# meituan/YOLOv6

Measured on NVIDIA H100. Metric: images/sec YOLOv6-S 640 bs32, higher is better.
Workload: dtype bf16

## Files before the change

### include/yv6.h

```cpp
#ifndef YV6_H_
#define YV6_H_

#include <stdint.h>

#ifdef __cplusplus
extern "C" {
#endif

#define YV6_ABI_VERSION 4

enum {
  YV6_OK = 0,
  YV6_ERR_ARG = -1,
  YV6_ERR_CUDA = -2,
  YV6_ERR_STATE = -3
};

enum { YV6_ACT_NONE = 0, YV6_ACT_RELU = 1, YV6_ACT_SILU = 2, YV6_ACT_SIGMOID = 3 };
enum { YV6_DT_BF16 = 0, YV6_DT_F32 = 1, YV6_DT_U8 = 2 };
#define YV6_PAD_SAME (-1000000)

typedef struct yv6_handle yv6_handle;

int yv6_create(int device, yv6_handle** out);
int yv6_destroy(yv6_handle* h);
const char* yv6_last_error(void);
int yv6_abi_version(void);

typedef struct yv6_conv_desc {
  const void* x;
  int32_t N, H, W, Cin;
  int32_t x_c_total;
  int64_t x_plane_stride;
  const void* w;
  int64_t w_plane_stride;
  const float* bias;
  int32_t Cout, kh, kw, stride, pad;
  int32_t act;
  void* y;
  int32_t y_dtype;
  int64_t y_img_stride, y_h_stride, y_w_stride;
  int64_t y_plane_stride;
  const void* res;
  float alpha;
  int64_t res_img_stride, res_h_stride, res_w_stride, res_plane_stride;
  int32_t nsplit;
  int32_t force_bw, force_bh, force_bi, force_bn, force_stages, force_grid;
  int32_t force_direct;
  int32_t force_halo;
  int32_t pad_w, out_h, out_w;
  int32_t force_groups;
  void* trace;
  int32_t stride_w;
  int32_t force_pair;
  int32_t pair_view;
  int32_t reserved0;
} yv6_conv_desc;

int yv6_conv_fwd(yv6_handle* h, const yv6_conv_desc* d, void* stream);
int yv6_conv_plan(yv6_handle* h, const yv6_conv_desc* d, int32_t* out10);
int yv6_conv_plan_host(int num_sms, int max_smem_optin, int max_clusters, const yv6_conv_desc* d, int32_t* out12);

typedef struct yv6_stem_desc {
  const void* x;
  int32_t x_dtype;
  float in_scale;
  int32_t N, H, W;
  const float* w;
  const float* bias;
  int32_t Cout, act;
  void* y;
  int64_t y_plane_stride;
  int32_t nsplit;
  int32_t fp32_math;
  int32_t force_sync_loads;
} yv6_stem_desc;
int yv6_stem_fwd(yv6_handle* h, const yv6_stem_desc* d, void* stream);

int yv6_sppf_pool(yv6_handle* h, void* buf, int32_t N, int32_t H, int32_t W, int32_t C, int32_t c_total,
                  int32_t nsplit, int64_t plane_stride, void* stream);

int yv6_head_decode(yv6_handle* h, const float* cls, const float* reg, float* out, int32_t B, int32_t nc,
                    int32_t reg_ch, int32_t nl, const int32_t* lvl_h, const int32_t* lvl_w,
                    const float* lvl_stride, void* stream);

int64_t yv6_nms_workspace_bytes(int32_t B, int32_t A, int32_t nc, int32_t multi_label);
int yv6_nms_batched(yv6_handle* h, const float* pred, int32_t B, int32_t A, int32_t nc, float conf_thres,
                    double iou_thres, int32_t agnostic, int32_t multi_label, const uint8_t* class_mask,
                    int32_t max_det, float* out, int32_t* out_count, int32_t* out_src, int32_t* overflow,
                    void* workspace, int64_t workspace_bytes, void* stream);

int yv6_nms_batched_head(yv6_handle* h, const float* cls, const float* reg, int32_t B, int32_t nc, int32_t reg_ch, int32_t nl,
                         const int32_t* lvl_h, const int32_t* lvl_w, const float* lvl_stride, float conf_thres, double iou_thres,
                         int32_t agnostic, int32_t multi_label, const uint8_t* class_mask, int32_t max_det, float* out,
                         int32_t* out_count, int32_t* out_src, int32_t* overflow, void* workspace, int64_t workspace_bytes,
                         void* stream);

int yv6_eval_boxes(yv6_handle* h, const float* det, const int32_t* count, const float* meta, int32_t B, int32_t max_det,
                   float* out, void* stream);

typedef struct yv6_pr_state {
  int32_t max_images, max_det, nc, confusion;
  float* conf; float* cls;
  uint16_t* correct;
  int32_t* ndet;
  int32_t* nt; int32_t* npred;
  int32_t* matrix;
  int32_t* flags;
} yv6_pr_state;
#define YV6_PR_OUT_SIZE(nc) ((int64_t)(nc) * 3010 + (int64_t)(nc) + ((int64_t)(nc) + 1) * ((int64_t)(nc) + 1) + 8)
int64_t yv6_pr_workspace_bytes(int32_t max_images, int32_t max_det);
int yv6_pr_match(yv6_handle* h, const yv6_pr_state* st, const float* det, const int32_t* count, int32_t B, int32_t max_det,
                 const float* targets, int32_t n_targets, const float* meta, int32_t H, int32_t W, const float* iouv,
                 int32_t first_image, void* stream);
int yv6_pr_metric(yv6_handle* h, const yv6_pr_state* st, int32_t n_images, const double* px, const double* x101, void* workspace,
                  int64_t workspace_bytes, double* out, void* stream);

#define YV6_LB_GEO 8
int yv6_letterbox(yv6_handle* h, const uint8_t* src, const int32_t* geo, int32_t B, int32_t H, int32_t W, uint8_t* dst,
                  void* stream);
int yv6_rescale_boxes(yv6_handle* h, const float* det, const int32_t* count, const int32_t* geo, int32_t B, int32_t max_det,
                      int32_t H, int32_t W, float* out, void* stream);

#define YV6_AUG_JOB 8
typedef struct {
  int64_t org;
  int32_t pitch;
  int32_t y0, y1, x0, x1;
  int32_t pad;
} yv6_aug_tile;
typedef struct {
  double minv[2][6];
  double mix_r;
  yv6_aug_tile tile[2][4];
  int32_t ch[2], cw[2];
  int32_t ntile[2];
  int32_t mixup, hsv, flipud, fliplr;
  uint8_t lut[3][256];
} yv6_aug_sample;
// ... 145 lines not shown
```

### yolov6_b200/_lib.py

```python
import ctypes as C
import os
import threading

_HERE = os.path.dirname(os.path.abspath(__file__))
LIB_PATH = os.path.join(_HERE, "libyolov6_b200.so")

ACT_NONE, ACT_RELU, ACT_SILU, ACT_SIGMOID = 0, 1, 2, 3
DT_BF16, DT_F32, DT_U8 = 0, 1, 2
PAD_SAME = -1000000
ACT_CODES = {None: ACT_NONE, "none": ACT_NONE, "relu": ACT_RELU, "silu": ACT_SILU, "sigmoid": ACT_SIGMOID}


class ConvDesc(C.Structure):
    _fields_ = [
        ("x", C.c_void_p), ("N", C.c_int32), ("H", C.c_int32), ("W", C.c_int32), ("Cin", C.c_int32),
        ("x_c_total", C.c_int32), ("x_plane_stride", C.c_int64),
        ("w", C.c_void_p), ("w_plane_stride", C.c_int64), ("bias", C.c_void_p),
        ("Cout", C.c_int32), ("kh", C.c_int32), ("kw", C.c_int32), ("stride", C.c_int32), ("pad", C.c_int32),
        ("act", C.c_int32),
        ("y", C.c_void_p), ("y_dtype", C.c_int32),
        ("y_img_stride", C.c_int64), ("y_h_stride", C.c_int64), ("y_w_stride", C.c_int64),
        ("y_plane_stride", C.c_int64),
        ("res", C.c_void_p), ("alpha", C.c_float),
        ("res_img_stride", C.c_int64), ("res_h_stride", C.c_int64), ("res_w_stride", C.c_int64),
        ("res_plane_stride", C.c_int64),
        ("nsplit", C.c_int32),
        ("force_bw", C.c_int32), ("force_bh", C.c_int32), ("force_bi", C.c_int32), ("force_bn", C.c_int32),
        ("force_stages", C.c_int32), ("force_grid", C.c_int32), ("force_direct", C.c_int32), ("force_halo", C.c_int32),
        ("pad_w", C.c_int32), ("out_h", C.c_int32), ("out_w", C.c_int32), ("force_groups", C.c_int32),
        ("trace", C.c_void_p), ("stride_w", C.c_int32), ("force_pair", C.c_int32), ("pair_view", C.c_int32), ("reserved0", C.c_int32),
    ]


class StemDesc(C.Structure):
    _fields_ = [
        ("x", C.c_void_p), ("x_dtype", C.c_int32), ("in_scale", C.c_float),
        ("N", C.c_int32), ("H", C.c_int32), ("W", C.c_int32),
        ("w", C.c_void_p), ("bias", C.c_void_p),
        ("Cout", C.c_int32), ("act", C.c_int32),
        ("y", C.c_void_p), ("y_plane_stride", C.c_int64), ("nsplit", C.c_int32), ("fp32_math", C.c_int32),
        ("force_sync_loads", C.c_int32),
    ]


class LossDesc(C.Structure):
    _fields_ = [
        ("pred_scores", C.c_void_p), ("pred_distri", C.c_void_p), ("anc_points", C.c_void_p), ("strides", C.c_void_p),
        ("gt", C.c_void_p), ("gt_idx", C.c_void_p), ("fg", C.c_void_p), ("norm", C.c_void_p),
        ("B", C.c_int32), ("A", C.c_int32), ("G", C.c_int32), ("nc", C.c_int32), ("reg_ch", C.c_int32),
        ("iou_type", C.c_int32),
        ("w_cls", C.c_double), ("w_iou", C.c_double), ("w_dfl", C.c_double), ("grad_scale", C.c_double),
        ("grad_scores", C.c_void_p), ("grad_distri", C.c_void_p), ("out", C.c_void_p),
        ("workspace", C.c_void_p), ("workspace_bytes", C.c_int64), ("norm_gt_zero", C.c_int32),
    ]


class WgradDesc(C.Structure):
    _fields_ = [
        ("x", C.c_void_p), ("N", C.c_int32), ("H", C.c_int32), ("W", C.c_int32), ("Cin", C.c_int32), ("x_c_total", C.c_int32),
        ("dy", C.c_void_p), ("Cout", C.c_int32), ("dy_c_total", C.c_int32),
        ("kh", C.c_int32), ("kw", C.c_int32), ("stride", C.c_int32), ("pad", C.c_int32),
        ("dw", C.c_void_p), ("force_ksplit", C.c_int32), ("force_taps", C.c_int32),
    ]


class BnDesc(C.Structure):
    _fields_ = [
        ("nb", C.c_int32), ("act", C.c_int32), ("C", C.c_int32), ("pixels", C.c_int64),
        ("x", C.c_void_p * 3), ("x_pitch", C.c_int64 * 3),
        ("mean", C.c_void_p * 3), ("invstd", C.c_void_p * 3), ("scale", C.c_void_p * 3), ("shift", C.c_void_p * 3),
        ("y", C.c_void_p), ("y_pitch", C.c_int64),
        ("dy", C.c_void_p), ("dy_pitch", C.c_int64),
        ("s1", C.c_void_p), ("s2", C.c_void_p * 3),
        ("dx", C.c_void_p * 3), ("dx_pitch", C.c_int64 * 3), ("accumulate", C.c_int32 * 3),
        ("res", C.c_void_p), ("res_pitch", C.c_int64), ("res_alpha", C.c_float),
        ("dres", C.c_void_p), ("dres_pitch", C.c_int64), ("dalpha", C.c_void_p),
        ("res_alpha_dev", C.c_void_p),
        ("work", C.c_void_p), ("counter", C.c_void_p), ("coef", C.c_void_p), ("zeroed", C.c_int32), ("dres_assign", C.c_int32),
    ]


class BnStatsDesc(C.Structure):
    _fields_ = [
        ("nb", C.c_int32), ("C", C.c_int32), ("pixels", C.c_int64),
        ("x", C.c_void_p * 3), ("x_pitch", C.c_int64 * 3),
        ("sums", C.c_void_p), ("counter", C.c_void_p), ("zeroed", C.c_int32),
        ("gamma", C.c_void_p * 3), ("beta", C.c_void_p * 3),
        ("running_mean", C.c_void_p * 3), ("running_var", C.c_void_p * 3),
        ("stats", C.c_void_p * 3),
        ("eps", C.c_float), ("momentum", C.c_float),
    ]


class XformSeg(C.Structure):
    _fields_ = [
        ("dst", C.c_void_p), ("src", C.c_void_p),
        ("n", C.c_int32 * 4), ("ds", C.c_int32 * 4), ("ss", C.c_int32 * 4),
        ("dst_dtype", C.c_int32), ("src_dtype", C.c_int32),
    ]


class PrState(C.Structure):
    _fields_ = [
        ("max_images", C.c_int32), ("max_det", C.c_int32), ("nc", C.c_int32), ("confusion", C.c_int32),
        ("conf", C.c_void_p), ("cls", C.c_void_p), ("correct", C.c_void_p), ("ndet", C.c_void_p),
        ("nt", C.c_void_p), ("npred", C.c_void_p), ("matrix", C.c_void_p), ("flags", C.c_void_p),
    ]


XF_F32, XF_F64, XF_BF16 = 0, 1, 2
XFORM_CHUNK = 4096


# ... 128 lines not shown
```

### yolov6_b200/csrc/yv6_conv_igemm.cu

```cuda
#include <algorithm>
#include <cstdarg>

#include "yv6_common.cuh"
#include "yv6_handle.h"
#include "yv6_wgmma.cuh"

namespace yv6 {

constexpr int kConvThreads = 384;
constexpr int kMaxStages = 12;
constexpr int kTileRows = 128;

struct ConvKParams {
  int32_t BW, BH, BI, rows;
  int32_t tiles_w, tiles_h, tiles_i, tiles_n, num_tiles;
  int32_t N, Ho, Wo, Cout, BN;
  int32_t taps, kw, stride, stride_w, pad, pad_w, Cin;
  int32_t cin_blocks, kb_elems, kb_bytes, ksteps;
  int32_t sbo_bytes, layout_type;
  int32_t npairs;
  int32_t stages, a_stage_bytes, b_stage_bytes;
  int32_t act, y_dtype, out_planes, res_planes;
  void* y;
  int64_t y_img_stride, y_h_stride, y_w_stride, y_plane_stride;
  const __nv_bfloat16* res;
  float alpha;
  int64_t res_img_stride, res_h_stride, res_w_stride, res_plane_stride;
  const float* bias;
  int32_t halo, a_stages, b_stages, b_resident;
  int32_t skip_cb;
  int32_t a_region_bytes, b_region_bytes;
  int32_t cpair, m_tiles, b_rows;
  int32_t fast_act;
};

constexpr int kHaloW = 10, kHaloH = 18;
template <bool S2>
struct HaloGeom {
  static constexpr int W = S2 ? 9 : kHaloW, H = S2 ? 33 : kHaloH, KW = S2 ? 2 : 3, TAPS = S2 ? 6 : 9, SH = S2 ? 2 : 1;
  static constexpr int kBytes = W * H * 128;
  static constexpr int kStageBytes = ((kBytes + 1023) / 1024) * 1024;
};
constexpr int kMaxAStages = 6, kMaxBStages = 40;

__host__ __device__ constexpr int stage_pitch(int bn) { return bn + 4; }
__host__ __device__ constexpr int staging_bytes(int bn) { return kTileRows * stage_pitch(bn) * 4; }

__device__ __forceinline__ void tma_load_3d(void* dst, const CUtensorMap* m, uint64_t* bar, int c0,
                                            int c1, int c2) {
  asm volatile(
      "cp.async.bulk.tensor.3d.shared::cluster.global.tile.mbarrier::complete_tx::bytes"
      " [%0], [%1, {%3, %4, %5}], [%2];" ::"r"(smem_u32(dst)),
      "l"(reinterpret_cast<uint64_t>(m)), "r"(smem_u32(bar)), "r"(c0), "r"(c1), "r"(c2)
      : "memory");
}
__device__ __forceinline__ void tma_load_3d_mc(void* dst, const CUtensorMap* m, uint64_t* bar, int c0, int c1, int c2,
                                               uint16_t mask) {
  asm volatile(
      "cp.async.bulk.tensor.3d.shared::cluster.global.mbarrier::complete_tx::bytes.multicast::cluster"
      " [%0], [%1, {%3, %4, %5}], [%2], %6;" ::"r"(smem_u32(dst)),
      "l"(reinterpret_cast<uint64_t>(m)), "r"(smem_u32(bar)), "r"(c0), "r"(c1), "r"(c2), "h"(mask)
      : "memory");
}
__device__ __forceinline__ void warpgroup_bar_sync(int wg) {
  asm volatile("bar.sync %0, 128;" ::"r"(1 + wg) : "memory");
}
__device__ __forceinline__ void producer_regs() { asm volatile("setmaxnreg.dec.sync.aligned.u32 40;"); }
__device__ __forceinline__ void consumer_regs() { asm volatile("setmaxnreg.inc.sync.aligned.u32 232;"); }

struct TileCoord {
  int w0, h0, i0, n0;
};
__device__ __forceinline__ TileCoord decode_tile(const ConvKParams& p, int tile) {
  TileCoord t;
  int nt = tile % p.tiles_n;
  int m = tile / p.tiles_n;
  int tw = m % p.tiles_w;
  m /= p.tiles_w;
  int th = m % p.tiles_h;
  int ti = m / p.tiles_h;
  t.w0 = tw * p.BW;
  t.h0 = th * p.BH;
  t.i0 = ti * p.BI;
  t.n0 = nt * p.BN;
  return t;
}

__device__ __forceinline__ TileCoord decode_unit(const ConvKParams& p, int unit, int rank) {
  TileCoord t;
  const int nt = unit % p.tiles_n;
  int m = (unit / p.tiles_n) * 2 + rank;
  t.n0 = nt * p.BN;
  if (m >= p.m_tiles) {
    t.w0 = 0;
    t.h0 = 0;
    t.i0 = p.N;
    return t;
  }
  const int tw = m % p.tiles_w;
  m /= p.tiles_w;
  const int th = m % p.tiles_h;
  const int ti = m / p.tiles_h;
  t.w0 = tw * p.BW;
  t.h0 = th * p.BH;
  t.i0 = ti * p.BI;
  return t;
}

__constant__ int kPairA[6] = {0, 1, 2, 0, 1, 0};
__constant__ int kPairB[6] = {2, 1, 0, 1, 0, 0};

__device__ __forceinline__ uint32_t pack_bf16x2(float a, float b) {
  __nv_bfloat162 v = __floats2bfloat162_rn(a, b);
  return *reinterpret_cast<uint32_t*>(&v);
}
// ... 70 lines not shown
    }
  } else {
#pragma unroll
    for (int j = 0; j < 16; ++j) v[j] = __uint_as_float(r[j]);
  }
  if (p.act == YV6_ACT_RELU) {
#pragma unroll
    for (int j = 0; j < 16; ++j) v[j] = fmaxf(v[j], 0.f);
  } else if (p.act == YV6_ACT_SILU) {
    if (p.fast_act) {
#pragma unroll
      for (int j = 0; j < 16; ++j) {
        const float h = 0.5f * v[j];
        v[j] = fmaf(h, tanh_fast(h), h);
      }
    } else {
#pragma unroll
      for (int j = 0; j < 16; ++j) v[j] = v[j] * rcp_ftz(1.f + ex2_ftz(-1.4426950408889634f * v[j]));
    }
  } else if (p.act == YV6_ACT_SIGMOID) {
#pragma unroll
    for (int j = 0; j < 16; ++j) v[j] = rcp_ftz(1.f + ex2_ftz(-1.4426950408889634f * v[j]));
  }
  if (p.res != nullptr && valid && ncol > 0) {
    for (int pl = 0; pl < p.res_planes; ++pl) {
      const __nv_bfloat16* rp = p.res + pl * p.res_plane_stride + roff + n;
      if (ncol == 16 && ((reinterpret_cast<uintptr_t>(rp) & 15) == 0)) {
        const uint4 q0 = __ldg(reinterpret_cast<const uint4*>(rp));
        const uint4 q1 = __ldg(reinterpret_cast<const uint4*>(rp) + 1);
        const uint32_t w[8] = {q0.x, q0.y, q0.z, q0.w, q1.x, q1.y, q1.z, q1.w};
#pragma unroll
        for (int j = 0; j < 8; ++j) {
          const __nv_bfloat162 b2 = *reinterpret_cast<const __nv_bfloat162*>(&w[j]);
          v[2 * j] += p.alpha * __low2float(b2);
          v[2 * j + 1] += p.alpha * __high2float(b2);
        }
      } else {
#pragma unroll
        for (int j = 0; j < 16; ++j)
          if (j < ncol) v[j] += p.alpha * __bfloat162float(rp[j]);
      }
    }
  }
}

template <int BN, int KSTEPS>
__device__ __forceinline__ void mma_kblock(float (&acc)[2][BN / 2], uint64_t ad, uint32_t a_hi, uint64_t bd, uint32_t scale_d) {
  wgmma_fence();
#pragma unroll
  for (int k = 0; k < KSTEPS; ++k) {
    const uint32_t sd = k == 0 ? scale_d : 1u;
    Wgmma<BN, 0, 0>::mma(acc[0], ad + (uint64_t)(2 * k), bd + (uint64_t)(2 * k), sd);
    Wgmma<BN, 0, 0>::mma(acc[1], ad + (uint64_t)(a_hi + 2 * k), bd + (uint64_t)(2 * k), sd);
  }
  wgmma_commit();
}

template <int BN, int MODE, bool CP>
__global__ void __launch_bounds__(kConvThreads, 1)
conv_igemm_kernel(const __grid_constant__ CUtensorMap tmA, const __grid_constant__ CUtensorMap tmB, const ConvKParams p) {
  extern __shared__ uint8_t smem_raw[];
  const uint32_t raw_addr = smem_u32(smem_raw);
  uint8_t* smem = smem_raw + ((1024u - (raw_addr & 1023u)) & 1023u);
  uint8_t* sA = smem;
  uint8_t* sB = smem + (size_t)p.a_region_bytes;
  float* sC = reinterpret_cast<float*>(sB + (size_t)p.b_region_bytes);
  uint64_t* bars = reinterpret_cast<uint64_t*>(reinterpret_cast<uint8_t*>(sC) + staging_bytes(BN));
  uint64_t* full = bars;
  uint64_t* empty = bars + kMaxStages;
  uint64_t* a_full = empty + kMaxStages;
  uint64_t* a_empty = a_full + kMaxAStages;
  uint64_t* b_full = a_empty + kMaxAStages;
  uint64_t* b_empty = b_full + kMaxBStages;
  uint64_t* mma_turn = b_empty + kMaxBStages;

  const int warp = threadIdx.x >> 5;
  const int lane = threadIdx.x & 31;
  constexpr bool HALO = (MODE != 0);
  constexpr bool BRES = (MODE == 2 || MODE == 4);
  using HG = HaloGeom<(MODE >= 3)>;
  const int rank = CP ? (int)cluster_ctarank() : 0;
  const int unit0 = CP ? (int)(blockIdx.x >> 1) : (int)blockIdx.x;
  const int ustep = CP ? (int)(gridDim.x >> 1) : (int)gridDim.x;
  auto coord = [&](int unit) { return CP ? decode_unit(p, unit, rank) : decode_tile(p, unit); };
  auto load_b = [&](uint8_t* dst, uint64_t* bar, int k, int n0, int plane) {
    if (CP) tma_load_3d_mc(dst + rank * p.b_rows * p.kb_bytes, &tmB, bar, k, n0 + rank * p.b_rows, plane, 3);
    else tma_load_3d(dst, &tmB, bar, k, n0, plane);
  };

  if (warp == 0) {
    if (lane == 0) {
      tma_prefetch_desc(&tmA);
      tma_prefetch_desc(&tmB);
    }
    constexpr int kRingSlots = 2 * kMaxStages + 2 * kMaxAStages + 2 * kMaxBStages;
    for (int i = lane; i < kRingSlots + 2; i += 32) {
      const bool is_b_empty = (i >= kMaxStages && i < 2 * kMaxStages) || (i >= 2 * kMaxStages + 2 * kMaxAStages + kMaxBStages && i < kRingSlots);
      mbar_init(&bars[i], i >= kRingSlots ? 128u : (is_b_empty && CP) ? 2u : 1u);
    }
    static_assert((kRingSlots + 2) * sizeof(uint64_t) <= 1024, "barriers overflow their 1 KB of shared memory");
    fence_mbar_init();
  }
  if (CP) cluster_sync_all();
  else __syncthreads();

  const int kblocks = p.npairs * p.taps * p.cin_blocks;

  if (warp < 4) {
    producer_regs();
    if (warp == 0) {
      if constexpr (HALO) {
        int sa = 0, sb = 0;
        uint32_t pha = 0, phb = 0;
        bool first = true;
        const uint32_t a_tx = (uint32_t)HG::kBytes, b_tx = (uint32_t)(BN * 128);
        for (int tile = unit0; tile < p.num_tiles; tile += ustep) {
          const TileCoord t = coord(tile);
          int slot = 0;
          for (int pi = 0; pi < p.npairs; ++pi) {
            const int pa = kPairA[6 - p.npairs + pi], pb = kPairB[6 - p.npairs + pi];
            for (int cb = 0; cb < p.cin_blocks; ++cb) {
              mbar_wait(&a_empty[sa], pha ^ 1);
              if (elect_one()) {
                mbar_expect_tx(&a_full[sa], a_tx);
                tma_load_5d(sA + (size_t)sa * HG::kStageBytes, &tmA, &a_full[sa], cb * 64, t.w0 - 1, t.h0 * HG::SH - 1, t.i0, pa);
              }
              __syncwarp();
              if (++sa == p.a_stages) { sa = 0; pha ^= 1; }
              for (int tap = 0; tap < HG::TAPS; ++tap) {
                if (HG::SH == 2 && (tap % HG::KW) == 0 && cb < p.skip_cb) continue;
                if constexpr (BRES) {
                  if (first && elect_one()) {
                    mbar_expect_tx(&b_full[slot], b_tx);
                    load_b(sB + (size_t)slot * p.b_stage_bytes, &b_full[slot], tap * p.Cin + cb * 64, t.n0, pb);
                  }
                  __syncwarp();
                } else {
                  mbar_wait(&b_empty[sb], phb ^ 1);
                  if (elect_one()) {
                    mbar_expect_tx(&b_full[sb], b_tx);
                    load_b(sB + (size_t)sb * p.b_stage_bytes, &b_full[sb], tap * p.Cin + cb * 64, t.n0, pb);
                  }
                  __syncwarp();
                  if (++sb == p.b_stages) { sb = 0; phb ^= 1; }
                }
                ++slot;
              }
            }
          }
          first = false;
        }
      } else {
        int stage = 0;
        uint32_t phase = 0;
        const uint32_t tx = (uint32_t)(p.rows * p.kb_bytes + BN * p.kb_bytes);
        for (int tile = unit0; tile < p.num_tiles; tile += ustep) {
          const TileCoord t = coord(tile);
          for (int pi = 0; pi < p.npairs; ++pi) {
            const int pa = kPairA[6 - p.npairs + pi], pb = kPairB[6 - p.npairs + pi];
            for (int tap = 0; tap < p.taps; ++tap) {
              const int r = tap / p.kw, s = tap - r * p.kw;
              const int cx = t.w0 * p.stride_w + s - p.pad_w;
              const int cy = t.h0 * p.stride + r - p.pad;
              for (int cb = 0; cb < p.cin_blocks; ++cb) {
                mbar_wait(&empty[stage], phase ^ 1);
                if (elect_one()) {
                  mbar_expect_tx(&full[stage], tx);
                  tma_load_5d(sA + (size_t)stage * p.a_stage_bytes, &tmA, &full[stage], cb * p.kb_elems, cx, cy, t.i0, pa);
                  load_b(sB + (size_t)stage * p.b_stage_bytes, &full[stage], tap * p.Cin + cb * p.kb_elems, t.n0, pb);
                }
                __syncwarp();
                if (++stage == p.stages) {
                  stage = 0;
                  phase ^= 1;
                }
              }
            }
          }
        }
      }
    }
  } else {
    consumer_regs();
    const int wg = (warp >> 2) - 1;
    const int ct = (int)threadIdx.x - 128 * (wg + 1);
    const bool arrive_lane = ct == 0;
    auto release_b = [&](uint64_t* bar) {
      mbar_arrive(bar);
      if (CP) mbar_arrive_cluster(bar, (uint32_t)(rank ^ 1));
    };
    auto skip_stages = [](int& s, uint32_t& ph, int n, int ring) {
      s += n;
      ph ^= (uint32_t)(s / ring) & 1u;
      s %= ring;
    };
    float acc[2][BN / 2];
    const uint32_t a_base = smem_u32(sA) >> 4, b_base = smem_u32(sB) >> 4;
    const int num_tiles = p.num_tiles, ksteps = p.ksteps, nstages = p.stages;
    const int pcs = p.npairs * p.cin_blocks;
    const int b_tile = p.npairs * (p.cin_blocks * HG::TAPS - (HG::SH == 2 ? (HG::TAPS / HG::KW) * p.skip_cb : 0));
    int stage = 0;
    uint32_t phase = 0;
    int sa = 0, sb = 0;
    uint32_t pha = 0, phb = 0, turn_ph = 0;
    bool first = true;
    float* sCw = sC + wg * 64 * stage_pitch(BN);
    for (int tile = unit0 + wg * ustep; tile < num_tiles; tile += 2 * ustep) {
      if (tile != unit0) {
        if constexpr (HALO) {
          skip_stages(sa, pha, pcs, p.a_stages);
          if (!BRES) skip_stages(sb, phb, b_tile, p.b_stages);
        } else {
          skip_stages(stage, phase, kblocks, nstages);
        }
        mbar_wait(&mma_turn[wg], turn_ph);
        turn_ph ^= 1;
      }
      if constexpr (HALO) {
        const uint32_t row_bytes = (uint32_t)(HG::W * 128 * HG::SH);
        const uint64_t desc_a = wgmma_desc(16u, row_bytes, 1u);
        const uint64_t desc_b = wgmma_desc(16u, 1024u, 1u);
        const uint32_t halo_step = (uint32_t)HG::kStageBytes >> 4, b_step = (uint32_t)p.b_stage_bytes >> 4;
        const uint32_t a_hi = 8u * (row_bytes >> 4);
        const int skip_cb = p.skip_cb, cin_blocks = p.cin_blocks, b_stages = p.b_stages;
        int slot = 0;
        uint32_t started = 0;
        int prev_sb = -1, prev_sa = -1;
        for (int pc = 0; pc < pcs; ++pc) {
          mbar_wait(&a_full[sa], pha);
          const uint32_t a0 = a_base + (uint32_t)sa * halo_step;
          const bool skip_s0 = (HG::SH == 2) && (pc % cin_blocks) < skip_cb;
#pragma unroll
          for (int tap = 0; tap < HG::TAPS; ++tap) {
            if (HG::SH == 2 && (tap % HG::KW) == 0 && skip_s0) continue;
            const int bs = BRES ? slot : sb;
            if (!BRES || first) mbar_wait(&b_full[bs], BRES ? 0u : phb);
            const uint64_t ad = desc_a | (uint64_t)(a0 + (uint32_t)((tap / HG::KW) * HG::W + (tap % HG::KW)) * 8u);
            const uint64_t bd = desc_b | (uint64_t)(b_base + (uint32_t)bs * b_step);
            mma_kblock<BN, 4>(acc, ad, a_hi, bd, started);
            started = 1u;
            if (!BRES || prev_sa >= 0) {
              wgmma_wait<1>();
              if (arrive_lane) {
                if (!BRES && prev_sb >= 0) release_b(&b_empty[prev_sb]);
                if (prev_sa >= 0) mbar_arrive(&a_empty[prev_sa]);
              }
              prev_sa = -1;
            }
            if (!BRES) {
              prev_sb = sb;
              if (++sb == b_stages) { sb = 0; phb ^= 1; }
            }
            ++slot;
          }
          prev_sa = sa;
          if (++sa == p.a_stages) { sa = 0; pha ^= 1; }
        }
        mbar_arrive(&mma_turn[wg ^ 1]);
        wgmma_wait<0>();
        if (arrive_lane) {
          if (!BRES && prev_sb >= 0) release_b(&b_empty[prev_sb]);
          if (prev_sa >= 0) mbar_arrive(&a_empty[prev_sa]);
        }
      } else {
        const uint64_t desc = wgmma_desc(16u, (uint32_t)p.sbo_bytes, (uint32_t)p.layout_type);
        const uint32_t a_step = (uint32_t)p.a_stage_bytes >> 4, b_step = (uint32_t)p.b_stage_bytes >> 4;
        const uint32_t a_hi = (uint32_t)(64 * p.kb_bytes) >> 4;
        int prev = -1;
        for (int kb = 0; kb < kblocks; ++kb) {
          mbar_wait(&full[stage], phase);
          const uint64_t ad = desc | (uint64_t)(a_base + (uint32_t)stage * a_step);
          const uint64_t bd = desc | (uint64_t)(b_base + (uint32_t)stage * b_step);
          const uint32_t scale_d = (uint32_t)(kb != 0);
          switch (ksteps) {
            case 1: mma_kblock<BN, 1>(acc, ad, a_hi, bd, scale_d); break;
            case 2: mma_kblock<BN, 2>(acc, ad, a_hi, bd, scale_d); break;
            default: mma_kblock<BN, 4>(acc, ad, a_hi, bd, scale_d); break;
          }
          wgmma_wait<1>();
          if (prev >= 0 && arrive_lane) release_b(&empty[prev]);
          prev = stage;
          if (++stage == nstages) {
            stage = 0;
            phase ^= 1;
          }
        }
        mbar_arrive(&mma_turn[wg ^ 1]);
        wgmma_wait<0>();
        if (prev >= 0 && arrive_lane) release_b(&empty[prev]);
      }
      wgmma_fence_operand(acc[0]);
      wgmma_fence_operand(acc[1]);
      first = false;

      const TileCoord t = coord(tile);
      constexpr int kChunks = BN / 16;
      const int r0 = (warp & 3) * 16 + (lane >> 2);
      const int c0 = 2 * (lane & 3);
#pragma unroll
      for (int h = 0; h < 2; ++h) {
        const int rows = min(64, p.rows - 64 * h);
        if (rows <= 0) break;
        warpgroup_bar_sync(wg);
#pragma unroll
        for (int j = 0; j < BN / 8; ++j) {
#pragma unroll
          for (int i = 0; i < 2; ++i) {
            *reinterpret_cast<float2*>(sCw + (r0 + 8 * i) * stage_pitch(BN) + 8 * j + c0) =
                make_float2(acc[h][4 * j + 2 * i], acc[h][4 * j + 2 * i + 1]);
          }
        }
        warpgroup_bar_sync(wg);
        for (int item = ct; item < rows * kChunks; item += 128) {
          const int lr = item / kChunks, ch = item - lr * kChunks;
          const int row = 64 * h + lr;
          const int n = t.n0 + 16 * ch;
          const int ncol = min(16, p.Cout - n);
          if (ncol <= 0) continue;
          const int bw = row % p.BW, tq = row / p.BW;
          const int bh = tq % p.BH, bi = tq / p.BH;
          const int img = t.i0 + bi, ho = t.h0 + bh, wo = t.w0 + bw;
          if (img >= p.N || ho >= p.Ho || wo >= p.Wo) continue;
          const int64_t off = (int64_t)img * p.y_img_stride + (int64_t)ho * p.y_h_stride + (int64_t)wo * p.y_w_stride;
          const int64_t roff = (int64_t)img * p.res_img_stride + (int64_t)ho * p.res_h_stride + (int64_t)wo * p.res_w_stride;
          const float4* src = reinterpret_cast<const float4*>(sCw + lr * stage_pitch(BN) + 16 * ch);
          uint32_t r[16];
#pragma unroll
          for (int q = 0; q < 4; ++q) {
            const float4 f = src[q];
            r[4 * q + 0] = __float_as_uint(f.x);
            r[4 * q + 1] = __float_as_uint(f.y);
            r[4 * q + 2] = __float_as_uint(f.z);
            r[4 * q + 3] = __float_as_uint(f.w);
          }
          float v[16];
          epilogue_math(p, nullptr, r, n, ncol, true, roff, v);
          store_chunk(p, off, n, ncol, v);
        }
      }
    }
  }
  if (CP) cluster_sync_all();
}

struct ConvPlan {
  ConvKParams k;
  int grid;
  size_t smem_bytes;
  CUtensorMapSwizzle swz;
};

constexpr int kBNs[4] = {32, 64, 96, 128};

static inline int ceil_div(int a, int b) { return (a + b - 1) / b; }

static int plan_conv(const yv6_handle* h, const yv6_conv_desc* d, ConvPlan* plan) {
  YV6_REQUIRE(d != nullptr, "conv: null descriptor");
  YV6_REQUIRE(d->x && d->w && d->y, "conv: null tensor pointer");
  YV6_REQUIRE(d->N > 0 && d->H > 0 && d->W > 0, "conv: bad input shape %dx%dx%d", d->N, d->H, d->W);
  YV6_REQUIRE(d->Cin > 0 && d->Cin % 16 == 0, "conv: Cin=%d must be a positive multiple of 16", d->Cin);
  YV6_REQUIRE(d->x_c_total >= d->Cin && d->x_c_total % 8 == 0, "conv: bad x_c_total=%d", d->x_c_total);
  YV6_REQUIRE(d->Cout > 0, "conv: Cout=%d", d->Cout);
  YV6_REQUIRE(d->kh >= 1 && d->kh <= 3 && d->kw >= 1 && d->kw <= 3, "conv: kernel %dx%d unsupported", d->kh, d->kw);
  YV6_REQUIRE(d->stride == 1 || d->stride == 2, "conv: stride %d unsupported", d->stride);
  YV6_REQUIRE(d->stride_w >= 0 && d->stride_w <= 2, "conv: stride_w %d unsupported", d->stride_w);
  const int stride_w = d->stride_w > 0 ? d->stride_w : d->stride;
  YV6_REQUIRE(d->nsplit == 1 || d->nsplit == 3, "conv: nsplit must be 1 or 3");
  YV6_REQUIRE((reinterpret_cast<uintptr_t>(d->x) & 15) == 0 && (reinterpret_cast<uintptr_t>(d->w) & 15) == 0,
              "conv: x / w must be 16-byte aligned");
  YV6_REQUIRE(d->y_dtype == YV6_DT_BF16 || d->y_dtype == YV6_DT_F32, "conv: bad y_dtype");

  ConvKParams& k = plan->k;
  memset(&k, 0, sizeof(k));
  k.N = d->N;
  const int pad_w = (d->pad_w == YV6_PAD_SAME) ? d->pad : d->pad_w;
  k.Ho = d->out_h > 0 ? d->out_h : (d->H + 2 * d->pad - d->kh) / d->stride + 1;
  k.Wo = d->out_w > 0 ? d->out_w : (d->W + 2 * pad_w - d->kw) / stride_w + 1;
  YV6_REQUIRE(k.Ho > 0 && k.Wo > 0, "conv: empty output");
// ... 35 lines not shown
        long tiles = (long)ceil_div(k.Wo, bw) * ceil_div(k.Ho, bh) * ceil_div(d->N, bi);
        if (best_tiles < 0 || tiles < best_tiles || (tiles == best_tiles && bw > bestw)) {
          best_tiles = tiles;
          bestw = bw;
          besth = bh;
          besti = bi;
        }
      }
    }
    for (int bw = 1; bw <= std::min(kTileRows, 256 / stride_w); bw <<= 1) {
      const int bh = kTileRows / bw;
      if (bh * d->stride > 256) continue;
      long tiles = (long)ceil_div(k.Wo, bw) * ceil_div(k.Ho, bh) * d->N;
      if (best_box_tiles < 0 || tiles < best_box_tiles || (tiles == best_box_tiles && bw > boxw)) {
        best_box_tiles = tiles;
        boxw = bw;
        boxh = bh;
      }
    }
    if (best_box_tiles > 0 && best_box_tiles * 100 <= best_tiles * 108 && d->force_bi == 0) {
      bestw = boxw;
      besth = boxh;
      besti = 1;
    }
    k.BW = bestw;
    k.BH = besth;
    k.BI = besti;
  }
  k.halo = 0;
  if (d->kh == 3 && d->kw == 3 && d->stride == 1 && stride_w == 1 && d->pad == 1 && pad_w == 1 && d->out_h == 0 && d->out_w == 0 &&
      d->Cin % 64 == 0 && d->force_bw == 0 && d->force_halo >= 0) {
    const long generic = (long)ceil_div(k.Wo, k.BW) * ceil_div(k.Ho, k.BH) * ceil_div(d->N, k.BI);
    const long halo_tiles = (long)ceil_div(k.Wo, 8) * ceil_div(k.Ho, 16) * d->N;
    if (d->force_halo > 0 || halo_tiles * 4 <= generic * 5) {
      k.halo = 1;
      k.BW = 8;
      k.BH = 16;
      k.BI = 1;
    }
  }
  k.skip_cb = 0;
  if (d->kh == 3 && d->kw == 2 && d->stride == 2 && stride_w == 1 && d->pad == 1 && pad_w == 1 && d->out_w == d->W && d->out_h == 0 &&
      d->Cin % 64 == 0 && d->force_bw == 0 && d->force_halo >= 0 && d->H % 2 == 0) {
    const long generic = (long)ceil_div(k.Wo, k.BW) * ceil_div(k.Ho, k.BH) * ceil_div(d->N, k.BI);
    const long halo_tiles = (long)ceil_div(k.Wo, 8) * ceil_div(k.Ho, 16) * d->N;
    if (d->force_halo > 0 || (halo_tiles * 4 <= generic * 5 && d->Cin <= 256)) {
      k.halo = 2;
      k.BW = 8;
      k.BH = 16;
      k.BI = 1;
      if (d->pair_view && (d->Cin / 2) % 64 == 0) k.skip_cb = d->Cin / 128;
    }
  }
  const long m_tiles = (long)ceil_div(k.Wo, k.BW) * ceil_div(k.Ho, k.BH) * ceil_div(d->N, k.BI);
  if (d->force_bn > 0) {
    YV6_REQUIRE(d->force_bn == 32 || d->force_bn == 64 || d->force_bn == 96 || d->force_bn == 128, "conv: force_bn must be 32, 64, 96 or 128");
    k.BN = d->force_bn;
  } else {
    double best_cost = -1;
    int best_bn = 0;
    for (int i = 3; i >= 0; --i) {
      const int bn = kBNs[i];
      if (bn < 64 && d->Cout > bn) continue;
      const long tiles = m_tiles * ceil_div(d->Cout, bn);
      const double waves = (double)ceil_div((int)std::min<long>(tiles, 1l << 30), h->num_sms);
      const double cost = waves * (bn + 48.0);
      if (best_cost < 0 || cost < best_cost - 1e-9) {
        best_cost = cost;
        best_bn = bn;
      }
    }
    k.BN = best_bn;
  }
  YV6_REQUIRE(k.BN >= 16, "conv: could not choose BN for Cout=%d", d->Cout);
  k.tiles_n = ceil_div(d->Cout, k.BN);
  k.rows = k.BW * k.BH * k.BI;
  k.tiles_w = ceil_div(k.Wo, k.BW);
  k.tiles_h = ceil_div(k.Ho, k.BH);
  k.tiles_i = ceil_div(d->N, k.BI);
  YV6_REQUIRE(m_tiles * k.tiles_n < (1l << 30), "conv: too many tiles");
  k.m_tiles = (int)m_tiles;
  k.cpair = (m_tiles >= 2 && h->max_clusters > 0 && d->force_pair > 0) ? 1 : 0;
  k.b_rows = k.cpair ? k.BN / 2 : k.BN;
  k.num_tiles = k.cpair ? (int)(((m_tiles + 1) / 2) * k.tiles_n) : (int)(m_tiles * k.tiles_n);

  k.a_stage_bytes = kTileRows * k.kb_bytes;
  k.b_stage_bytes = ((k.BN * k.kb_bytes + 1023) / 1024) * 1024;
  const int budget = h->max_smem_optin - 1024 - 1024 - staging_bytes(k.BN);
  if (k.halo) {
    const int halo_stage = (k.halo == 2) ? HaloGeom<true>::kStageBytes : HaloGeom<false>::kStageBytes;
    const int min_a = (k.halo == 2) ? 2 : 3;
    const int b_tiles = (k.halo == 2) ? k.npairs * (k.cin_blocks * 6 - 3 * k.skip_cb) : k.npairs * k.cin_blocks * 9;
    k.b_resident = (k.tiles_n == 1 && b_tiles <= kMaxBStages && d->force_stages == 0 &&
                    (long)b_tiles * k.b_stage_bytes + min_a * halo_stage <= budget) ? 1 : 0;
    if (k.b_resident) {
      k.b_stages = b_tiles;
      k.a_stages = std::min(kMaxAStages, (budget - b_tiles * k.b_stage_bytes) / halo_stage);
    } else {
      k.a_stages = (k.halo == 1 && budget - 3 * halo_stage >= 3 * k.b_stage_bytes) ? 3 : 2;
      k.b_stages = std::min(kMaxBStages, (budget - k.a_stages * halo_stage) / k.b_stage_bytes);
      if (d->force_stages > 0) k.b_stages = std::min(k.b_stages, std::max(2, d->force_stages));
    }
    YV6_REQUIRE(k.a_stages >= 2 && k.b_stages >= 2, "conv(halo): not enough shared memory");
    k.stages = k.b_stages;
    k.a_region_bytes = k.a_stages * halo_stage;
    k.b_region_bytes = k.b_stages * k.b_stage_bytes;
  } else {
    const int stage_bytes = k.a_stage_bytes + k.b_stage_bytes;
    int stages = std::min(kMaxStages, budget / stage_bytes);
    if (d->force_stages > 0) stages = std::min(stages, d->force_stages);
    YV6_REQUIRE(stages >= 2, "conv: not enough shared memory for a 2-stage pipeline");
    k.stages = stages;
    k.a_region_bytes = stages * k.a_stage_bytes;
    k.b_region_bytes = stages * k.b_stage_bytes;
  }
  plan->smem_bytes = (size_t)k.a_region_bytes + k.b_region_bytes + staging_bytes(k.BN) + 1024 + 1024;

  k.act = d->act;
  k.y_dtype = d->y_dtype;
  k.fast_act = (d->y_dtype == YV6_DT_BF16 && d->nsplit != 3) ? 1 : 0;
  k.out_planes = (d->nsplit == 3 && d->y_dtype == YV6_DT_BF16) ? 3 : 1;
  k.res_planes = (d->nsplit == 3) ? 3 : 1;
  k.y = d->y;
  k.y_img_stride = d->y_img_stride;
  k.y_h_stride = d->y_h_stride;
  k.y_w_stride = d->y_w_stride;
  k.y_plane_stride = d->y_plane_stride;
  k.res = reinterpret_cast<const __nv_bfloat16*>(d->res);
  k.alpha = d->alpha;
  k.res_img_stride = d->res_img_stride;
  k.res_h_stride = d->res_h_stride;
  k.res_w_stride = d->res_w_stride;
  k.res_plane_stride = d->res_plane_stride;
  k.bias = d->bias;

  if (k.cpair) {
    int clusters = std::min(k.num_tiles, h->max_clusters);
    if (d->force_grid > 0) clusters = std::min(k.num_tiles, std::max(1, d->force_grid / 2));
    plan->grid = 2 * clusters;
  } else {
    plan->grid = std::min(k.num_tiles, h->num_sms);
    if (d->force_grid > 0) plan->grid = std::min(k.num_tiles, d->force_grid);
  }
  return YV6_OK;
}

}

using namespace yv6;

using ConvKernelFn = void (*)(const CUtensorMap, const CUtensorMap, const ConvKParams);
#define YV6_CONV_MODES(BN, CP)                                                                                      \
  {conv_igemm_kernel<BN, 0, CP>, conv_igemm_kernel<BN, 1, CP>, conv_igemm_kernel<BN, 2, CP>, conv_igemm_kernel<BN, 3, CP>, \
   conv_igemm_kernel<BN, 4, CP>}
static const ConvKernelFn kConvKernels[2][4][5] = {
    {YV6_CONV_MODES(32, false), YV6_CONV_MODES(64, false), YV6_CONV_MODES(96, false), YV6_CONV_MODES(128, false)},
    {YV6_CONV_MODES(32, true), YV6_CONV_MODES(64, true), YV6_CONV_MODES(96, true), YV6_CONV_MODES(128, true)}};
#undef YV6_CONV_MODES

static int conv_configure(yv6_handle* h) {
  if (h->configured & YV6_CFG_CONV) return YV6_OK;
  for (int c = 0; c < 2; ++c)
    for (int b = 0; b < 4; ++b)
      for (int m = 0; m < 5; ++m)
        YV6_CHECK_CUDA(cudaFuncSetAttribute(kConvKernels[c][b][m], cudaFuncAttributeMaxDynamicSharedMemorySize, (int)h->max_smem_optin));
  cudaLaunchConfig_t cfg;
  memset(&cfg, 0, sizeof(cfg));
  cfg.gridDim = dim3((unsigned)(2 * h->num_sms));
  cfg.blockDim = dim3(kConvThreads);
  cfg.dynamicSmemBytes = 200 * 1024;
  cudaLaunchAttribute attr[1];
  attr[0].id = cudaLaunchAttributeClusterDimension;
  attr[0].val.clusterDim.x = 2;
  attr[0].val.clusterDim.y = 1;
  attr[0].val.clusterDim.z = 1;
  cfg.attrs = attr;
  cfg.numAttrs = 1;
  int n = 0;
  if (cudaOccupancyMaxActiveClusters(&n, kConvKernels[1][3][0], &cfg) != cudaSuccess) {
    (void)cudaGetLastError();
    n = 0;
  }
  h->max_clusters = std::min(n, h->num_sms / 2);
  h->configured |= YV6_CFG_CONV;
  return YV6_OK;
}

extern "C" int yv6_conv_plan(yv6_handle* h, const yv6_conv_desc* d, int32_t* out8) {
  yv6_device_guard _dev(h);
  YV6_REQUIRE(h != nullptr && out8 != nullptr, "conv_plan: null argument");
  { const int rc0 = conv_configure(h); if (rc0 != YV6_OK) return rc0; }
  ConvPlan plan;
  int rc = plan_conv(h, d, &plan);
  if (rc != YV6_OK) return rc;
  out8[0] = plan.k.BW;
  out8[1] = plan.k.BH;
  out8[2] = plan.k.BI;
  out8[3] = plan.k.BN;
  out8[4] = plan.k.kb_elems;
// ... 17 lines not shown
  ConvPlan plan;
  int rc = plan_conv(&fake, d, &plan);
  if (rc != YV6_OK) return rc;
  YV6_REQUIRE(plan.smem_bytes <= (size_t)max_smem_optin, "conv_plan_host: plan needs %zu bytes of shared memory, device offers %d",
              plan.smem_bytes, max_smem_optin);
  out12[0] = plan.k.BW;
  out12[1] = plan.k.BH;
  out12[2] = plan.k.BI;
  out12[3] = plan.k.BN;
  out12[4] = plan.k.kb_elems;
  out12[5] = plan.k.stages;
  out12[6] = plan.grid;
  out12[7] = plan.k.num_tiles;
  out12[8] = plan.k.halo;
  out12[9] = (plan.k.halo ? plan.k.a_stages * 100 + plan.k.b_resident : 0) + 10 * plan.k.cpair;
  out12[10] = (int32_t)plan.smem_bytes;
  out12[11] = kConvThreads;
  return YV6_OK;
}

extern "C" int yv6_conv_fwd(yv6_handle* h, const yv6_conv_desc* d, void* stream) {
  yv6_device_guard _dev(h);
  YV6_REQUIRE(h != nullptr, "conv_fwd: null handle");
  { const int rc0 = conv_configure(h); if (rc0 != YV6_OK) return rc0; }
  ConvPlan plan;
  int rc = plan_conv(h, d, &plan);
  if (rc != YV6_OK) return rc;
  const ConvKParams& k = plan.k;
  YV6_REQUIRE(h->encode_tiled != nullptr, "conv_fwd: cuTensorMapEncodeTiled unavailable (no CUDA driver?)");

  CUtensorMap tmA, tmB;
  {
    const uint64_t planes = (d->nsplit == 3) ? 3 : 1;
    cuuint64_t dims[5] = {(cuuint64_t)d->Cin, (cuuint64_t)d->W, (cuuint64_t)d->H, (cuuint64_t)d->N, planes};
    const uint64_t pix = (uint64_t)d->x_c_total * 2;
    uint64_t plane_stride = (d->nsplit == 3) ? (uint64_t)d->x_plane_stride * 2
                                             : (uint64_t)d->N * d->H * d->W * pix;
    YV6_REQUIRE(plane_stride % 16 == 0, "conv: x_plane_stride must be a multiple of 8 elements");
    cuuint64_t strides[4] = {pix, pix * d->W, pix * d->W * d->H, plane_stride};
    cuuint32_t box[5] = {(cuuint32_t)k.kb_elems, (cuuint32_t)(k.BW * k.stride_w), (cuuint32_t)(k.BH * d->stride),
                         (cuuint32_t)k.BI, 1};
    cuuint32_t estr[5] = {1, (cuuint32_t)k.stride_w, (cuuint32_t)d->stride, 1, 1};
    if (k.halo) {
      box[1] = (k.halo == 2) ? HaloGeom<true>::W : HaloGeom<false>::W;
      box[2] = (k.halo == 2) ? HaloGeom<true>::H : HaloGeom<false>::H;
      estr[1] = estr[2] = 1;
    }
    CUresult cr = h->encode_tiled(&tmA, CU_TENSOR_MAP_DATA_TYPE_BFLOAT16, 5, const_cast<void*>(d->x), dims,
                                  strides, box, estr, CU_TENSOR_MAP_INTERLEAVE_NONE, plan.swz,
                                  CU_TENSOR_MAP_L2_PROMOTION_L2_256B, CU_TENSOR_MAP_FLOAT_OOB_FILL_NONE);
    if (cr != CUDA_SUCCESS) {
      yv6_set_error("conv: cuTensorMapEncodeTiled(A) failed with %d (C=%d W=%d H=%d N=%d box=%u,%u,%u,%u)", (int)cr,
                    d->Cin, d->W, d->H, d->N, box[0], box[1], box[2], box[3]);
      return YV6_ERR_CUDA;
    }
  }
  {
    const uint64_t planes = (d->nsplit == 3) ? 3 : 1;
    const uint64_t ktot = (uint64_t)k.taps * d->Cin;
    cuuint64_t dims[3] = {ktot, (cuuint64_t)d->Cout, planes};
    uint64_t plane_stride = (d->nsplit == 3) ? (uint64_t)d->w_plane_stride * 2 : ktot * 2 * d->Cout;
    YV6_REQUIRE(plane_stride % 16 == 0, "conv: w_plane_stride must be a multiple of 8 elements");
    cuuint64_t strides[2] = {ktot * 2, plane_stride};
    cuuint32_t box[3] = {(cuuint32_t)k.kb_elems, (cuuint32_t)k.b_rows, 1};
    cuuint32_t estr[3] = {1, 1, 1};
    CUresult cr = h->encode_tiled(&tmB, CU_TENSOR_MAP_DATA_TYPE_BFLOAT16, 3, const_cast<void*>(d->w), dims,
                                  strides, box, estr, CU_TENSOR_MAP_INTERLEAVE_NONE, plan.swz,
                                  CU_TENSOR_MAP_L2_PROMOTION_L2_256B, CU_TENSOR_MAP_FLOAT_OOB_FILL_NONE);
    if (cr != CUDA_SUCCESS) {
      yv6_set_error("conv: cuTensorMapEncodeTiled(B) failed with %d", (int)cr);
      return YV6_ERR_CUDA;
    }
  }

  const int mode = k.halo ? (k.halo == 2 ? 3 : 1) + (k.b_resident ? 1 : 0) : 0;
  const int bn_idx = k.BN == 32 ? 0 : k.BN == 64 ? 1 : k.BN == 96 ? 2 : 3;
  ConvKernelFn fn = kConvKernels[k.cpair][bn_idx][mode];
  cudaLaunchConfig_t cfg;
  memset(&cfg, 0, sizeof(cfg));
  cfg.gridDim = dim3((unsigned)plan.grid);
  cfg.blockDim = dim3((unsigned)kConvThreads);
  cfg.dynamicSmemBytes = plan.smem_bytes;
  cfg.stream = (cudaStream_t)stream;
  cudaLaunchAttribute attr[1];
  if (k.cpair) {
    attr[0].id = cudaLaunchAttributeClusterDimension;
    attr[0].val.clusterDim.x = 2;
    attr[0].val.clusterDim.y = 1;
    attr[0].val.clusterDim.z = 1;
    cfg.attrs = attr;
    cfg.numAttrs = 1;
  }
  YV6_CHECK_CUDA(cudaLaunchKernelEx(&cfg, fn, tmA, tmB, k));
  YV6_CHECK_CUDA(cudaGetLastError());
  return YV6_OK;
}
```

Measured before the change: 5973.

## Share B tiles across consumer warpgroups and enable programmatic dependent launch

Adds an opt-in 'share' mode for halo convs where both consumer warpgroups process the two M-halves of one unit. A separate producer warp fills A while warp 0 loads B once for both, and the B empty barriers count two arrivals. Separately, every conv launch now sets programmatic stream serialization and calls griddepcontrol wait/launch_dependents, so a kernel's prologue can overlap the previous kernel's tail. Share mode only runs when force_share is set, but the PDL change applies to all launches.

```diff
diff --git a/include/yv6.h b/include/yv6.h
--- a/include/yv6.h
+++ b/include/yv6.h
@@ -54,7 +54,7 @@
   int32_t stride_w;
   int32_t force_pair;
   int32_t pair_view;
-  int32_t reserved0;
+  int32_t force_share;
 } yv6_conv_desc;
 
 int yv6_conv_fwd(yv6_handle* h, const yv6_conv_desc* d, void* stream);
diff --git a/yolov6_b200/_lib.py b/yolov6_b200/_lib.py
--- a/yolov6_b200/_lib.py
+++ b/yolov6_b200/_lib.py
@@ -28,7 +28,7 @@
         ("force_bw", C.c_int32), ("force_bh", C.c_int32), ("force_bi", C.c_int32), ("force_bn", C.c_int32),
         ("force_stages", C.c_int32), ("force_grid", C.c_int32), ("force_direct", C.c_int32), ("force_halo", C.c_int32),
         ("pad_w", C.c_int32), ("out_h", C.c_int32), ("out_w", C.c_int32), ("force_groups", C.c_int32),
-        ("trace", C.c_void_p), ("stride_w", C.c_int32), ("force_pair", C.c_int32), ("pair_view", C.c_int32), ("reserved0", C.c_int32),
+        ("trace", C.c_void_p), ("stride_w", C.c_int32), ("force_pair", C.c_int32), ("pair_view", C.c_int32), ("force_share", C.c_int32),
     ]
 
 
diff --git a/yolov6_b200/csrc/yv6_conv_igemm.cu b/yolov6_b200/csrc/yv6_conv_igemm.cu
--- a/yolov6_b200/csrc/yv6_conv_igemm.cu
+++ b/yolov6_b200/csrc/yv6_conv_igemm.cu
@@ -31,6 +31,7 @@
   int32_t skip_cb;
   int32_t a_region_bytes, b_region_bytes;
   int32_t cpair, m_tiles, b_rows;
+  int32_t share;
   int32_t fast_act;
 };
 
@@ -267,7 +268,10 @@
   const int rank = CP ? (int)cluster_ctarank() : 0;
   const int unit0 = CP ? (int)(blockIdx.x >> 1) : (int)blockIdx.x;
   const int ustep = CP ? (int)(gridDim.x >> 1) : (int)gridDim.x;
-  auto coord = [&](int unit) { return CP ? decode_unit(p, unit, rank) : decode_tile(p, unit); };
+  const bool share = MODE == 1 && !CP && p.share != 0;
+  auto coord = [&](int unit, int half) {
+    return CP ? decode_unit(p, unit, rank) : share ? decode_unit(p, unit, half) : decode_tile(p, unit);
+  };
   auto load_b = [&](uint8_t* dst, uint64_t* bar, int k, int n0, int plane) {
     if (CP) tma_load_3d_mc(dst + rank * p.b_rows * p.kb_bytes, &tmB, bar, k, n0 + rank * p.b_rows, plane, 3);
     else tma_load_3d(dst, &tmB, bar, k, n0, plane);
@@ -281,37 +285,44 @@
     constexpr int kRingSlots = 2 * kMaxStages + 2 * kMaxAStages + 2 * kMaxBStages;
     for (int i = lane; i < kRingSlots + 2; i += 32) {
       const bool is_b_empty = (i >= kMaxStages && i < 2 * kMaxStages) || (i >= 2 * kMaxStages + 2 * kMaxAStages + kMaxBStages && i < kRingSlots);
-      mbar_init(&bars[i], i >= kRingSlots ? 128u : (is_b_empty && CP) ? 2u : 1u);
+      mbar_init(&bars[i], i >= kRingSlots ? 128u : (is_b_empty && (CP || share)) ? 2u : 1u);
     }
     static_assert((kRingSlots + 2) * sizeof(uint64_t) <= 1024, "barriers overflow their 1 KB of shared memory");
     fence_mbar_init();
   }
   if (CP) cluster_sync_all();
   else __syncthreads();
+  asm volatile("griddepcontrol.wait;" ::: "memory");
+  asm volatile("griddepcontrol.launch_dependents;" ::: "memory");
 
   const int kblocks = p.npairs * p.taps * p.cin_blocks;
 
   if (warp < 4) {
     producer_regs();
-    if (warp == 0) {
+    if (warp == 0 || (share && warp == 1)) {
       if constexpr (HALO) {
+        const bool fills_a = !share || warp == 1, fills_b = warp == 0;
         int sa = 0, sb = 0;
         uint32_t pha = 0, phb = 0;
         bool first = true;
         const uint32_t a_tx = (uint32_t)HG::kBytes, b_tx = (uint32_t)(BN * 128);
         for (int tile = unit0; tile < p.num_tiles; tile += ustep) {
-          const TileCoord t = coord(tile);
+          const TileCoord t = coord(tile, 0);
           int slot = 0;
           for (int pi = 0; pi < p.npairs; ++pi) {
             const int pa = kPairA[6 - p.npairs + pi], pb = kPairB[6 - p.npairs + pi];
             for (int cb = 0; cb < p.cin_blocks; ++cb) {
-              mbar_wait(&a_empty[sa], pha ^ 1);
-              if (elect_one()) {
-                mbar_expect_tx(&a_full[sa], a_tx);
-                tma_load_5d(sA + (size_t)sa * HG::kStageBytes, &tmA, &a_full[sa], cb * 64, t.w0 - 1, t.h0 * HG::SH - 1, t.i0, pa);
+              for (int half = 0; fills_a && half < (share ? 2 : 1); ++half) {
+                const TileCoord ta = half ? coord(tile, 1) : t;
+                mbar_wait(&a_empty[sa], pha ^ 1);
+                if (elect_one()) {
+                  mbar_expect_tx(&a_full[sa], a_tx);
+                  tma_load_5d(sA + (size_t)sa * HG::kStageBytes, &tmA, &a_full[sa], cb * 64, ta.w0 - 1, ta.h0 * HG::SH - 1, ta.i0, pa);
+                }
+                __syncwarp();
+                if (++sa == p.a_stages) { sa = 0; pha ^= 1; }
               }
-              __syncwarp();
-              if (++sa == p.a_stages) { sa = 0; pha ^= 1; }
+              if (!fills_b) continue;
               for (int tap = 0; tap < HG::TAPS; ++tap) {
                 if (HG::SH == 2 && (tap % HG::KW) == 0 && cb < p.skip_cb) continue;
                 if constexpr (BRES) {
@@ -340,7 +351,7 @@
         uint32_t phase = 0;
         const uint32_t tx = (uint32_t)(p.rows * p.kb_bytes + BN * p.kb_bytes);
         for (int tile = unit0; tile < p.num_tiles; tile += ustep) {
-          const TileCoord t = coord(tile);
+          const TileCoord t = coord(tile, 0);
           for (int pi = 0; pi < p.npairs; ++pi) {
             const int pa = kPairA[6 - p.npairs + pi], pb = kPairB[6 - p.npairs + pi];
             for (int tap = 0; tap < p.taps; ++tap) {
@@ -390,8 +401,8 @@
     uint32_t pha = 0, phb = 0, turn_ph = 0;
     bool first = true;
     float* sCw = sC + wg * 64 * stage_pitch(BN);
-    for (int tile = unit0 + wg * ustep; tile < num_tiles; tile += 2 * ustep) {
-      if (tile != unit0) {
+    for (int tile = share ? unit0 : unit0 + wg * ustep; tile < num_tiles; tile += share ? ustep : 2 * ustep) {
+      if (!share && tile != unit0) {
         if constexpr (HALO) {
           skip_stages(sa, pha, pcs, p.a_stages);
           if (!BRES) skip_stages(sb, phb, b_tile, p.b_stages);
@@ -412,6 +423,7 @@
         uint32_t started = 0;
         int prev_sb = -1, prev_sa = -1;
         for (int pc = 0; pc < pcs; ++pc) {
+          if (share) skip_stages(sa, pha, wg, p.a_stages);
           mbar_wait(&a_full[sa], pha);
           const uint32_t a0 = a_base + (uint32_t)sa * halo_step;
           const bool skip_s0 = (HG::SH == 2) && (pc % cin_blocks) < skip_cb;
@@ -440,8 +452,9 @@
           }
           prev_sa = sa;
           if (++sa == p.a_stages) { sa = 0; pha ^= 1; }
+          if (share) skip_stages(sa, pha, 1 - wg, p.a_stages);
         }
-        mbar_arrive(&mma_turn[wg ^ 1]);
+        if (!share) mbar_arrive(&mma_turn[wg ^ 1]);
         wgmma_wait<0>();
         if (arrive_lane) {
           if (!BRES && prev_sb >= 0) release_b(&b_empty[prev_sb]);
@@ -478,7 +491,7 @@
       wgmma_fence_operand(acc[1]);
       first = false;
 
-      const TileCoord t = coord(tile);
+      const TileCoord t = coord(tile, wg);
       constexpr int kChunks = BN / 16;
       const int r0 = (warp & 3) * 16 + (lane >> 2);
       const int c0 = 2 * (lane & 3);
@@ -680,7 +693,6 @@
   k.m_tiles = (int)m_tiles;
   k.cpair = (m_tiles >= 2 && h->max_clusters > 0 && d->force_pair > 0) ? 1 : 0;
   k.b_rows = k.cpair ? k.BN / 2 : k.BN;
-  k.num_tiles = k.cpair ? (int)(((m_tiles + 1) / 2) * k.tiles_n) : (int)(m_tiles * k.tiles_n);
 
   k.a_stage_bytes = kTileRows * k.kb_bytes;
   k.b_stage_bytes = ((k.BN * k.kb_bytes + 1023) / 1024) * 1024;
@@ -713,6 +725,9 @@
     k.b_region_bytes = stages * k.b_stage_bytes;
   }
   plan->smem_bytes = (size_t)k.a_region_bytes + k.b_region_bytes + staging_bytes(k.BN) + 1024 + 1024;
+  const long units = ((m_tiles + 1) / 2) * k.tiles_n;
+  k.share = (k.halo == 1 && !k.b_resident && !k.cpair && m_tiles >= 2 && d->force_share > 0) ? 1 : 0;
+  k.num_tiles = (k.cpair || k.share) ? (int)units : (int)(m_tiles * k.tiles_n);
 
   k.act = d->act;
   k.y_dtype = d->y_dtype;
@@ -896,14 +911,17 @@
   cfg.blockDim = dim3((unsigned)kConvThreads);
   cfg.dynamicSmemBytes = plan.smem_bytes;
   cfg.stream = (cudaStream_t)stream;
-  cudaLaunchAttribute attr[1];
+  cudaLaunchAttribute attr[2];
+  attr[0].id = cudaLaunchAttributeProgrammaticStreamSerialization;
+  attr[0].val.programmaticStreamSerializationAllowed = 1;
+  cfg.attrs = attr;
+  cfg.numAttrs = 1;
   if (k.cpair) {
-    attr[0].id = cudaLaunchAttributeClusterDimension;
-    attr[0].val.clusterDim.x = 2;
-    attr[0].val.clusterDim.y = 1;
-    attr[0].val.clusterDim.z = 1;
-    cfg.attrs = attr;
-    cfg.numAttrs = 1;
+    attr[1].id = cudaLaunchAttributeClusterDimension;
+    attr[1].val.clusterDim.x = 2;
+    attr[1].val.clusterDim.y = 1;
+    attr[1].val.clusterDim.z = 1;
+    cfg.numAttrs = 2;
   }
   YV6_CHECK_CUDA(cudaLaunchKernelEx(&cfg, fn, tmA, tmB, k));
   YV6_CHECK_CUDA(cudaGetLastError());
```

Measured after the change: 5986 (median of 6 runs). No clear change (+0.2%).
